# AlerianEmperor/CaitlynRenderer

Measured on AMD Instinct MI355X. Metric: Mray/s (primary+1 bounce) at 1920x1080, higher is better.
Workload: dtype f32

## Files before the change

caitlynrenderer_amd/csrc/crt_device.cpp:

```cpp
#include <hip/hip_runtime.h>
#include <dlfcn.h>

#include <algorithm>
#include <atomic>
#include <chrono>
#include <cmath>
#include <cstdio>
#include <cstdlib>
#include <cstring>
#include <memory>
#include <mutex>
#include <thread>
#include <new>
#include <string>
#include <vector>

#include "../../include/crt.h"
#include "crt_error.hpp"
#include "device_build.hpp"
#include "host/cwbvh.hpp"
#include "host/flatnode_link.hpp"
#include "host/refit_core.hpp"
#include "instances.hpp"
#include "instances_bind.hpp"
// ... 154 lines not shown
    uint32_t* d_counts = nullptr;
    uint32_t bank = 0;
    bool counts_clean = false;
    uint32_t* counts() const { return d_counts + (size_t)bank * kCounters; }
    uint32_t* h_counts = nullptr;
    bool frame_buffers_ready = false;

    crt_camera cam{};
    bool have_camera = false;
    uint32_t jitter = 1;
    bool count_visits = false;
    bool count_batched = false;
    unsigned long long* d_visit_totals = nullptr;
    unsigned long long* h_visit_totals = nullptr;

    float4* d_t_rays = nullptr; float4* d_t_hits = nullptr; uint32_t* d_t_stats = nullptr; size_t t_cap = 0;

    std::vector<EventSpan> spans;
    int n_spans = 0;
    crt_frame_stats stats{};
    bool stats_pending = false;
    bool stats_from_frame = false;
    bool stats_counted = false;
    uint32_t tri_min = 2;
    uint32_t inplace_shadow = 3;
    uint32_t accel = 0;
    uint32_t refill_min = 8;
    uint32_t trace_pool = 64;
    uint32_t trace_occupancy = 8;
    uint32_t oversubscribe = 0;
    bool special_materials = false;
    uint32_t waves_per_workgroup = 1;
    uint32_t lanes_per_ray = 8;
    uint32_t* d_overflow = nullptr;
    float4* d_lfinal = nullptr;
    uint32_t ray_bins = 0;
    bool rows_padded = false;
    bool rays_doubled = false;
    uint32_t* d_bins = nullptr;
    float bounds_lo[3] = {0.f, 0.f, 0.f}, bounds_hi[3] = {1.f, 1.f, 1.f};
    uint32_t* bin_count(uint32_t seg) const { return d_bins + (size_t)seg * CRT_RAY_BINS; }
    uint32_t* bin_cap(uint32_t par, uint32_t seg) const { return d_bins + (size_t)(17 + par * 17 + seg) * CRT_RAY_BINS; }
    uint32_t* bin_off(uint32_t par, uint32_t seg) const { return d_bins + (size_t)(17 * 3 + par * 17 + seg) * CRT_RAY_BINS; }
    uint32_t* bin_start(uint32_t seg) const { return d_bins + (size_t)17 * 5 * CRT_RAY_BINS + (size_t)seg * (CRT_RAY_BINS + 1u); }
    uint32_t* bin_ovf(uint32_t seg) const { return d_bins + (size_t)17 * 5 * CRT_RAY_BINS + (size_t)17 * (CRT_RAY_BINS + 1u) + (size_t)seg * 32u; }
    static size_t bins_words() { return (size_t)17 * 5 * CRT_RAY_BINS + (size_t)17 * (CRT_RAY_BINS + 1u) + 17u * 32u; }
    uint32_t debug_fail_batch_alloc = 0;
    uint32_t batch_cap = 1;
    uint32_t samples_in_stats = 1;
    uint32_t timing = 0;
    bool timing_accumulate = false;

    std::vector<crt_scene*> peers;
    crt_scene* primary = nullptr;
    std::vector<std::pair<size_t, size_t>> scene_bufs;
    uint32_t shard_rank = 0, shard_world = 1;
    uint32_t streams = 1;
    bool shares_scene = false;
    std::vector<float*> d_gather;
    std::vector<uint2*> d_peer_tiles;
    std::vector<hipEvent_t> ev_peer;
    void* rccl_lib = nullptr;
    std::vector<void*> rccl_comms;
    uint32_t gather_transport = 0;
    float last_gather_ms = 0.f;

// ... 876 lines not shown
    else if (!std::strcmp(name, "persistent")) s->persistent = value ? 1u : 0u;
    else if (!std::strcmp(name, "sort_shadow")) s->sort_shadow = value ? 1u : 0u;
#ifdef CRT_EXPERIMENTS
    else if (!std::strcmp(name, "trace_occupancy")) s->trace_occupancy = (uint32_t)std::max(1, value);
    else if (!std::strcmp(name, "oversubscribe")) s->oversubscribe = (uint32_t)std::max(0, value);
    else if (!std::strcmp(name, "waves_per_workgroup")) {
        if (value != 1 && value != 2 && value != 4) return fail(CRT_ERR_INVALID, "crt_set_option: waves_per_workgroup is 1, 2 or 4");
        s->waves_per_workgroup = (uint32_t)value;
    }
#else
    else if (!std::strcmp(name, "trace_occupancy") || !std::strcmp(name, "oversubscribe") || !std::strcmp(name, "waves_per_workgroup")) {
        const bool is_default = !std::strcmp(name, "waves_per_workgroup") ? value == 1 : !std::strcmp(name, "oversubscribe") ? value == 0 : true;
        if (!is_default) return fail(CRT_ERR_INVALID, std::string("crt_set_option: ") + name + " is an experimental variant: this library was built without CRT_EXPERIMENTS");
    }
#endif
    else if (!std::strcmp(name, "streams")) {
        if (value < 0 || value > 4) return fail(CRT_ERR_INVALID, "crt_set_option: streams is 0 (pick for me) or 1..4");
        if (value == 0) value = s->info.n_nodes8 < 64 ? 3 : s->max_depth > 1 ? 2 : 1;
        if (s->primary) return fail(CRT_ERR_INVALID, "crt_set_option: streams is set on the scene, not on a replica");
        if ((uint32_t)value == s->streams) return CRT_OK;
        if (s->streams == 1u && !s->peers.empty())
            return fail(CRT_ERR_INVALID, "crt_set_option: streams is for a scene on one device (crt_set_devices already deals its tiles to several)");
        const std::vector<int32_t> ids((size_t)value, (int32_t)s->device);
        const int rc = set_devices_of_shard(s, ids.data(), (uint32_t)value, s->tile ? s->tile : 16u, s->shard_rank, s->shard_world);
        if (rc) return rc;
        s->streams = (uint32_t)value;
        return CRT_OK;
    }
    else if (!std::strcmp(name, "wave_samples")) s->wave_samples = value < 0 ? 0u : std::min<uint32_t>(3u, (uint32_t)value);
    else if (!std::strcmp(name, "wide_first")) s->wide_first = value < 0 ? 0u : std::min<uint32_t>(2u, (uint32_t)value);
    else if (!std::strcmp(name, "lanes_per_ray")) {
        if (value != 1 && value != 8) return fail(CRT_ERR_INVALID, "crt_set_option: lanes_per_ray is 1 or 8");
        s->lanes_per_ray = (uint32_t)value;
    }
    else if (!std::strcmp(name, "inplace_shadow")) {
        if (value < 0 || value > 3) return fail(CRT_ERR_INVALID, "crt_set_option: inplace_shadow is 1 (in place), 0 (every segment's shadow rays deferred), 2 (bounce segments' deferred) or 3 (pick for me)");
        s->inplace_shadow = (uint32_t)value;
    }
    else if (!std::strcmp(name, "adaptive_tiles")) { s->adaptive_tiles = value ? 1u : 0u; if (value) s->tile_state = crt_scene::TILES_WANT; }
    else if (!std::strcmp(name, "accel")) {
        if (value < 0 || value > 2) return fail(CRT_ERR_INVALID, "crt_set_option: accel is 0 (CWBVH), 1 (BVH2, reference order) or 2 (BVH2, lowest-id ties)");
        if (value != 0 && !s->d_bvh2) return fail(CRT_ERR_INVALID, "crt_set_option: the scene was created without a BVH2 (desc.bvh)");
        if (value != 0 && s->special_materials)
            return fail(CRT_ERR_INVALID, "crt_set_option: the BVH2 frame mode is the shipped shader, which is Lambert only; this scene has Mirror / Disney materials");
        s->accel = (uint32_t)value;
    }
    else if (!std::strcmp(name, "timing")) s->timing = (uint32_t)std::max(0, value);
    else if (!std::strcmp(name, "timing_accumulate")) {
        HIPCHK(hipSetDevice(s->device));
        HIPCHK(hipStreamSynchronize(s->stream));
        s->timing_accumulate = value != 0;
        s->n_spans = 0;
        const size_t want = value > 0 ? (size_t)std::min(value, 1 << 14) : 0;
        try { if (s->spans.size() < want) s->spans.resize(want); } catch (const std::exception&) { return fail(CRT_ERR_NOMEM, "crt_set_option: out of host memory (timing spans)"); }
    }
    else if (!std::strcmp(name, "ray_bins")) s->ray_bins = (uint32_t)std::min(5, std::max(0, value));
    else if (!std::strcmp(name, "debug_fail_batch_alloc")) {
        if (value >= 2 && (size_t)(value - 2) < s->peers.size()) s->peers[(size_t)(value - 2)]->debug_fail_batch_alloc = 1u;
        else s->debug_fail_batch_alloc = value == 1 ? 1u : 0u;
        if (value == 0) for (crt_scene* p : s->peers) p->debug_fail_batch_alloc = 0u;
        return CRT_OK;
    }
    else if (!std::strcmp(name, "tri_min")) s->tri_min = (uint32_t)std::min(64, std::max(0, value));
    else if (!std::strcmp(name, "refill_min")) s->refill_min = (uint32_t)std::min(65, std::max(1, value));
    else if (!std::strcmp(name, "trace_pool")) {
        if (value != 64 && value != 128 && value != 256) return fail(CRT_ERR_INVALID, "crt_set_option: trace_pool is 64, 128 or 256");
// ... 211 lines not shown
            HIPCHK(hipMemcpyAsync(s->d_tile_order, s->h_tile_order, nt * sizeof(uint32_t), hipMemcpyHostToDevice, s->stream));
            HIPCHK(hipEventRecord(s->ev_tile_order, s->stream));
            s->tile_order_uploading = true;
            s->tile_state = crt_scene::TILES_DONE;
        }
        ++s->frames_since_tile_measure;
        if (s->tile_state == crt_scene::TILES_WANT && !s->count_visits && (!s->tiles_measured_once || s->frames_since_tile_measure >= 16u)) {
            s->tiles_measured_once = true;
            s->frames_since_tile_measure = 0;
            HIPCHK(hipMemsetAsync(s->d_tile_cost, 0, s->n_local_tiles * sizeof(uint32_t), s->stream));
            measure_tiles = true;
        }
    }
    s->bank ^= 1u;
    if (s->accel == 0u) { const int prc = ensure_planes(s); if (prc) return prc; }
    if (!s->counts_clean) HIPCHK(hipMemsetAsync(s->d_counts, 0, 2 * kCounters * sizeof(uint32_t), s->stream));
    s->counts_clean = false;
    uint32_t* const cnt = s->counts();

    for (uint32_t b = 0; b < s->max_depth; ++b) {
        crt::SegmentArgs sa{};
        sa.nodes = s->d_nodes; sa.planes = s->d_planes; sa.tris = s->d_tris; sa.triangles = s->d_triangles; sa.normals = s->d_normals;
        sa.materials = s->d_materials; sa.lights = s->d_lights; sa.n_lights = (int32_t)s->n_lights;
        sa.stack_entries = s->stack_entries;
        sa.texcoords = s->d_texcoords; sa.textures = s->d_textures;
        sa.tex_width = s->tex_width; sa.tex_height = s->tex_height; sa.n_textures = s->n_textures;
        sa.f = f;
        sa.sub_capacity = s->sub_capacity;
        const bool bvh2 = s->accel != 0u;
        const bool small_tree = s->info.n_nodes8 < 64;
        const bool inplace = b < first_deferred;
        sa.tri_min = small_tree ? 0u : s->tri_min;
        sa.lanes_log2 = s->lanes_per_ray >= 8u ? 3u : s->lanes_per_ray >= 4u ? 2u : s->lanes_per_ray >= 2u ? 1u : 0u;
        sa.nodes2 = s->d_bvh2; sa.tris2 = s->d_tris2; sa.stack_entries2 = s->bvh2_stack; sa.tie = s->accel == 2u ? 1u : 0u;
        const bool bins = uses_ray_bins(s);
        const uint32_t Qe = 8u * s->sub_capacity;
        if (bins && b + 1 < s->max_depth) {
            crt::RayBins& o = sa.bins_out;
            o.count = s->bin_count(b + 1); o.cap = s->bin_cap(s->bank, b + 1); o.off = s->bin_off(s->bank, b + 1);
            o.ovf_count = s->bin_ovf(b + 1); o.ovf_base = Qe;
            o.per_lane = s->ray_bins == 2u ? 1u : s->ray_bins == 3u ? (b > 0 ? 1u : 0u) : s->ray_bins == 4u ? 2u : s->ray_bins == 5u ? (b > 0 ? 2u : 0u) : 0u;
            for (int k = 0; k < 3; ++k) {
                const float ext = s->bounds_hi[k] - s->bounds_lo[k];
                o.origin[k] = s->bounds_lo[k];
                o.scale[k] = ext > 0.f ? 8.0f / ext : 0.f;
            }
        }
        if (bins && b > 0) { sa.bin_start = s->bin_start(b); sa.bin_off_in = s->bin_off(s->bank, b); sa.ovf_base_in = Qe; }
        sa.rays_in = s->d_rays[b & 1]; sa.count_in = cnt + counter_index(b, 0, 0);
        sa.rays_next = s->d_rays[(b + 1) & 1]; sa.count_next = cnt + counter_index(b + 1, 0, 0);
        sa.count_shadow = cnt + counter_index(b, 1, 0);
        if (!inplace) {
            const uint32_t r = b - first_deferred;
            sa.shadow = s->d_nee + 2 * (size_t)r * 8u * s->sub_capacity;
            sa.contrib = s->d_contrib + (size_t)r * n_paths;
            sa.slot_first = (uint32_t)((size_t)r * n_paths);
            sa.slot_bit = 1u << (8u + b);
        }
        sa.pb = s->pb; sa.sum = s->d_sum;
        sa.last_segment = (b + 1 == s->max_depth) ? 1u : 0u;
        sa.visit_totals = s->d_visit_totals;
        sa.overflow = s->d_overflow;
        if (b == 0) { sa.zero_counts = s->d_counts + (size_t)(s->bank ^ 1u) * kCounters; sa.n_zero = kCounters; }
        sa.l_final = folds ? s->d_lfinal : nullptr;
        sa.tile_cost = (b == 0 && measure_tiles) ? s->d_tile_cost : nullptr;
        sa.n_samples = b == 0 ? n_samples : 1u;
// ... 473 lines not shown

}

void crt_scene::drop_peers() {
    if (!rccl_comms.empty() && g_rccl.destroy)
        for (void* c : rccl_comms) if (c) (void)g_rccl.destroy(c);
    rccl_comms.clear();
    for (crt_scene* p : peers) delete p;
    peers.clear();
    if (!d_gather.empty() || !d_peer_tiles.empty() || !ev_peer.empty()) (void)hipSetDevice(device);
    for (float* b : d_gather) if (b) (void)hipFree(b);
    for (uint2* b : d_peer_tiles) if (b) (void)hipFree(b);
    for (hipEvent_t e : ev_peer) if (e) (void)hipEventDestroy(e);
    d_gather.clear(); d_peer_tiles.clear(); ev_peer.clear();
}

static int replicate_scene(const crt_scene* src, int device, crt_scene** out) {
    *out = nullptr;
    HIPCHK(hipSetDevice(device));
    std::unique_ptr<crt_scene> owner(new (std::nothrow) crt_scene);
    crt_scene* r = owner.get();
    if (!r) return fail(CRT_ERR_NOMEM, "crt_set_devices: out of memory");
    r->device = device;
    hipDeviceProp_t prop;
    if (hipGetDeviceProperties(&prop, device) == hipSuccess) r->n_cu = prop.multiProcessorCount;
    HIPCHK(hipStreamCreateWithFlags(&r->stream, hipStreamNonBlocking));
    r->width = src->width; r->height = src->height; r->max_depth = src->max_depth; r->n_lights = src->n_lights;
    r->tex_width = src->tex_width; r->tex_height = src->tex_height; r->n_textures = src->n_textures;
    r->info = src->info; r->bvh2_stack = src->bvh2_stack; r->stack_entries = src->stack_entries; r->special_materials = src->special_materials;
    r->cam = src->cam; r->have_camera = src->have_camera; r->jitter = src->jitter;
    r->tri_min = src->tri_min; r->inplace_shadow = src->inplace_shadow; r->accel = src->accel; r->refill_min = src->refill_min; r->trace_pool = src->trace_pool; r->count_visits = src->count_visits;
    r->count_batched = src->count_batched;
    r->trace_occupancy = src->trace_occupancy; r->oversubscribe = src->oversubscribe; r->waves_per_workgroup = src->waves_per_workgroup;
    r->lanes_per_ray = src->lanes_per_ray; r->bounce_refill = src->bounce_refill; r->refill_pool = src->refill_pool; r->shadow_pool = src->shadow_pool; r->shadow_refill_min = src->shadow_refill_min; r->shadow_waves = src->shadow_waves; r->persistent = src->persistent; r->sort_shadow = src->sort_shadow;
    r->wave_samples = src->wave_samples; r->wide_first = src->wide_first; r->adaptive_tiles = src->adaptive_tiles; r->timing = src->timing;
    r->ray_bins = src->ray_bins; r->rows_padded = src->rows_padded;
    for (int k = 0; k < 3; ++k) { r->bounds_lo[k] = src->bounds_lo[k]; r->bounds_hi[k] = src->bounds_hi[k]; }
    r->scene_bufs = src->scene_bufs;
    r->shares_scene = device == src->device;
    if (device != src->device) {
        int can = 0;
        if (hipDeviceCanAccessPeer(&can, device, src->device) == hipSuccess && can) (void)hipDeviceEnablePeerAccess(src->device, 0);
        (void)hipGetLastError();
    }
    for (const auto& b : src->scene_bufs) {
        const void* from = *reinterpret_cast<void* const*>(reinterpret_cast<const char*>(src) + b.first);
        void** to = reinterpret_cast<void**>(reinterpret_cast<char*>(r) + b.first);
        if (!from) continue;
        if (device == src->device) { *to = const_cast<void*>(from); continue; }
        hipError_t e = hipMalloc(to, b.second ? b.second : 16);
        if (e != hipSuccess) return fail(CRT_ERR_NOMEM, std::string("crt_set_devices: hipMalloc: ") + hipGetErrorString(e));
        if (b.second) HIPCHK(hipMemcpyPeer(*to, device, from, src->device, b.second));
    }
    int rc = finish_scene_setup(r);
    if (rc) return rc;
    *out = owner.release();
    return CRT_OK;
}

int crt_set_devices(crt_scene* s, const int32_t* devices, uint32_t n_devices, uint32_t tile) {
    if (s && s->inst && n_devices > 1)
        return fail(CRT_ERR_INVALID, "crt_set_devices: an instanced scene renders on the one device its crt_instances handle lives on");
    const int rc = set_devices_of_shard(s, devices, n_devices, tile, 0u, 1u);
    if (rc == CRT_OK) { s->shard_rank = 0u; s->shard_world = 1u; }
    return rc;
}

// ... 508 lines not shown
```

caitlynrenderer_amd/csrc/rt_kernels.hip:

```cpp
#include <hip/hip_runtime.h>
#include <hip/hip_ext.h>
#include <stdint.h>

#include <type_traits>
#include <stdlib.h>

#include <algorithm>

#include "rt_kernels.hpp"
#include "rt_math.hpp"
#include "host/flatnode_link.hpp"
#include "rt_traverse.hpp"

namespace crt {

#define CRT_INF 1e9f
#define CRT_EPS 1e-4f
#define CRT_PI 3.1415926f
#define CRT_PI2 6.2831853f


#ifdef CRT_ISA_MARKS
#define CRT_MARK(name) asm volatile("; CRT_MARK " name)
#else
// ... 698 lines not shown
                const uint32_t hitmask = node8_intersect(n0, n1, n2, n3, n4, o, inv, negx, negy, negz, oct4, tmax);
                cur.x = n1.x;
                tg.x = n1.y;
                cur.y = (hitmask & 0xff000000u) | (n0.w >> 24);
                tg.y = hitmask & 0x00ffffffu;
                }
                CRT_MARK("node_end");
            }
            while (tg.y) {
                CRT_MARK("tri_begin");
                const int b = 31 - __builtin_clz(tg.y);
                tg.y &= ~(1u << b);
                const uint32_t ti = tg.x + (uint32_t)b;
                const float4* tp = tri_rows(tris, ti);
                const float4 ta = tp[0], tb = tp[1], tc = tp[2];
                if (STATS) { ++n_tris; count_wave_step(w_tris); }
                float u, v, t;
                if (mt_test(ta, tb, tc, o, d, u, v, t) && t < tmax) { hit_tri = (int)ti; tg.y = 0u; cur.y = 0u; sp = 0; }
                CRT_MARK("tri_end");
            }
            if (!(cur.y & 0xff000000u) && sp != 0) { --sp; cur = stk[sp * 64]; }
        }
    }
    busy = (cur.y & 0xff000000u) != 0u;
    CRT_MARK("loop_end");
    HitState out;
    out.t = tmax; out.tri = hit_tri;
    if (regroup)
        group_phase<true, STATS, false>(nodes, tris, base, stack_entries, overflow, busy, o, d, tmax, -1, cur, tg, sp, tri_min, out, n_nodes, n_tris, w_nodes, w_tris,
                                        V3(0.f, 0.f, 0.f));
    return out.tri >= 0;
}

__device__ __forceinline__ void flush_visit_totals(unsigned long long* totals, uint32_t nn, uint32_t nt, uint32_t wn = 0u, uint32_t wt = 0u) {
    unsigned long long a = nn, b = nt, c = wn, d = wt;
    for (int off = 32; off > 0; off >>= 1) {
        a += __shfl_down(a, off);
        b += __shfl_down(b, off);
        c += __shfl_down(c, off);
        d += __shfl_down(d, off);
    }
    if ((threadIdx.x & 63u) == 0) {
        if (a) atomicAdd(&totals[0], a);
        if (b) atomicAdd(&totals[1], b);
        if (c) atomicAdd(&totals[4], c);
        if (d) atomicAdd(&totals[5], d);
    }
}

template <bool ANY, bool STATS>
__global__ void __launch_bounds__(CRT_TRACE_BLOCK) k_trace(TraceArgs a) {
    extern __shared__ uint2 s_lds[];
    const WaveId wid = wave_id(false, false, a.pool_split_log2);
    const uint32_t lane = wid.lane, wave = wid.wave;
    uint2* stk = s_lds + (size_t)wid.lds_wave * (a.stack_entries + CRT_HIT_SLOTS) * 64u + lane;
    const uint32_t n = a.count_ptr ? *a.count_ptr : a.n;
    uint32_t nn_total = 0, nt_total = 0;
    CRT_CHUNK_LOOP(it) {
        const uint32_t v = static_pool_chunk<true>(wid, nullptr, n, it);
        if (v == CRT_NO_WORK) break;
        const uint32_t pool = 256u >> a.pool_split_log2;
        const uint32_t first = dense_pool_first(v, wave) + wid.sub * pool;
        if (first >= n) continue;
        const uint32_t last = first + pool < n ? first + pool : n;
        uint32_t nn = 0, nt = 0, wn_unused = 0, wt_unused = 0;
        uint32_t nn0 = 0, nt0 = 0;
// ... 292 lines not shown
    float dy = (2.0f * ty - 1.0f) + jy;
    dx = dx * f.aspect_tan;
    dy = dy * f.tan_fov;
    const vec3 right = V3(f.cam_right[0], f.cam_right[1], f.cam_right[2]);
    const vec3 up = V3(f.cam_up[0], f.cam_up[1], f.cam_up[2]);
    const vec3 fwd = V3(f.cam_forward[0], f.cam_forward[1], f.cam_forward[2]);
    d = normalize((right * dx + up * dy) + fwd);
    o = V3(f.cam_pos[0], f.cam_pos[1], f.cam_pos[2]);
}

typedef const __attribute__((address_space(4))) SegmentArgs* KArgs;
__device__ __forceinline__ RayBins load_bins(KArgs k) {
    RayBins b;
    b.count = k->bins_out.count; b.cap = k->bins_out.cap; b.off = k->bins_out.off; b.ovf_count = k->bins_out.ovf_count;
    b.ovf_base = k->bins_out.ovf_base; b.per_lane = k->bins_out.per_lane;
    for (int i = 0; i < 3; ++i) { b.origin[i] = k->bins_out.origin[i]; b.scale[i] = k->bins_out.scale[i]; }
    return b;
}
__device__ __forceinline__ KArgs kernarg_here() {
    KArgs p = (KArgs)__builtin_amdgcn_kernarg_segment_ptr();
    asm volatile("" : "+s"(p));
    return p;
}

#ifndef CRT_SEG_OCC
#define CRT_SEG_OCC 6
#endif
#ifndef CRT_SEG_OCC_DEFERRED
#define CRT_SEG_OCC_DEFERRED 8
#endif
#ifndef CRT_SEG_OCC_FIRST
#define CRT_SEG_OCC_FIRST 6
#endif
#ifndef CRT_SEG_OCC_BATCH
#define CRT_SEG_OCC_BATCH 5
#endif

template <bool FIRST, bool STATS, bool TEX, bool PRETRACED, bool INPLACE, bool BVH2 = false, bool MAT = false, bool BATCH = false, bool WIDE = false, bool ONE = false,
          bool INST = false>
__global__ void __launch_bounds__(CRT_TRACE_BLOCK, ((WIDE || ONE) ? CRT_SEG_OCC_FIRST : (BATCH || STATS) ? CRT_SEG_OCC_BATCH : (!FIRST && !INPLACE && !PRETRACED) ? CRT_SEG_OCC_DEFERRED : CRT_SEG_OCC)) k_segment(std::conditional_t<INST, InstSegmentArgs, SegmentArgs> a) {
    extern __shared__ uint2 s_lds[];
    constexpr bool UNI_K = FIRST;
    const bool wave_samples = BATCH && !WIDE && !ONE && a.wave_samples == 1u;
    const bool lane_samples = BATCH && (ONE || a.wave_samples == 2u);
    const WaveId wid = wave_id(wave_samples, lane_samples);
    const uint32_t lane = wid.lane, wave = wid.wave;
    const uint32_t wave_stride = (a.stack_entries + CRT_HIT_SLOTS) * 64u;
    uint2* stk = s_lds + (size_t)wid.lds_wave * wave_stride + lane;
    int* stk2 = reinterpret_cast<int*>(s_lds) + (size_t)wid.lds_wave * a.stack_entries2 * 64u + lane;
    const float4* const recs = BVH2 ? a.tris2 : a.tris;
    const FrameArgs& f = a.f;
    uint32_t nn = 0, nt = 0, nn_any = 0, nt_any = 0;
    uint32_t wn = 0, wt = 0, wn_any = 0, wt_any = 0;
    uint32_t n_hits = 0;
    uint32_t nu = 0, nu_any = 0;
    if (FIRST && a.zero_counts && blockIdx.x == 0)
        for (uint32_t i = threadIdx.x; i < a.n_zero; i += blockDim.x) a.zero_counts[i] = 0u;
    CRT_CHUNK_LOOP(it) {
        uint32_t v;
        if (!FIRST && a.bin_start) {
            const uint32_t n_chunks = queue_chunks(a.count_in[0]), per_group = (n_chunks + 7u) >> 3;
            const uint32_t grp = wid.vblock & 7u, c = (wid.vblock >> 3) + it * (wid.vgrid >> 3);
            v = (c < per_group && grp * per_group + c < n_chunks) ? (grp << 28) | (grp * per_group + c) : CRT_NO_WORK;
        } else {
            v = static_chunk<FIRST>(wid, a.count_in, f.n_local_pixels, it);
        }
        if (v == CRT_NO_WORK) break;
        const uint32_t g = v >> 28;
        uint32_t* const count_shadow = a.count_shadow + g * CRT_COUNTER_STRIDE;
        uint32_t* const count_next = a.count_next + g * CRT_COUNTER_STRIDE;
        float4* const shadow_q = a.shadow + 2 * (size_t)g * a.sub_capacity;
        float4* const next_q = a.rays_next + 2 * (size_t)g * a.sub_capacity;
        uint32_t e, n;
// ... 293 lines not shown
                            sdir = (ou * dl.x + ov * dl.y) + n * dl.z;
                            bsdf_pdf = __fdiv_rn(dot(sdir, n) * 1.0f, CRT_PI);
                            T = T * albedo;
                        }
                        if (go_on) {
                            if (INPLACE && pending) pend_pdf = bsdf_pdf;
                            else if (INPLACE || FIRST) ka->pb.L[pix] = make_float4(L.x, L.y, L.z, bsdf_pdf);
                            else reinterpret_cast<float*>(ka->pb.L + pix)[3] = bsdf_pdf;
                            ka->pb.T[pix] = make_float4(T.x, T.y, T.z, __uint_as_float((disney ? 2u : 0u) | slot_mask));
                            ka->pb.seed[pix] = make_float2(sx, sy);
                            emit_next = true;
                            finished = false;
                            nx0 = make_float4(hit_point.x, hit_point.y, hit_point.z, CRT_INF);
                            nx1 = make_float4(sdir.x, sdir.y, sdir.z, __uint_as_float(pix));
                        }
                    }
                }
            }
        }
        if (ka->bins_out.count) {
            const RayBins bins_out = load_bins(ka);
            CRT_MARK("loop_begin bins");
            uint32_t* const tab = wave_stride * 8u >= 3072u ? reinterpret_cast<uint32_t*>(s_lds + (size_t)wid.lds_wave * wave_stride) : nullptr;
            const uint32_t ni = bin_append(bins_out, emit_next, ray_bin_key(bins_out, nx0, nx1), tab);
            if (emit_next) { ka->rays_next[2 * (size_t)ni] = nx0; ka->rays_next[2 * (size_t)ni + 1] = nx1; }
            CRT_MARK("loop_end");
        } else {
            const uint32_t ni = wave_append(emit_next, count_next);
            if (emit_next) { next_q[2 * (size_t)ni] = nx0; next_q[2 * (size_t)ni + 1] = nx1; }
        }
        if (INPLACE) {
            const bool lanes_walks = !BVH2 && (ONE || (a.lanes_log2 != 0u && a.tri_min != 0u));
            if (FIRST && lanes_walks) {
                const bool occluded = traverse_any_then_groups<STATS, UNI_K>(a.nodes, a.tris, stk - lane, (int)a.stack_entries, a.overflow, pending, V3(sh0.x, sh0.y, sh0.z),
                                                                      V3(sh1.x, sh1.y, sh1.z), sh0.w, a.tri_min, a.lanes_log2, nn_any, nt_any, wn_any, wt_any, &nu_any, a.planes);
                if (pending && !occluded) L = L + V3(sh2.x, sh2.y, sh2.z);
            } else if (lanes_walks) {
                HitState shh;
                walk_batch<true, STATS, false, UNI_K>(a.nodes, a.tris, stk - lane, (int)a.stack_entries, a.overflow, pending, V3(sh0.x, sh0.y, sh0.z), V3(sh1.x, sh1.y, sh1.z),
                                               sh0.w, a.tri_min, a.lanes_log2, shh, nn_any, nt_any, wn_any, wt_any, V3(0.f, 0.f, 0.f), &nu_any, a.planes);
                if (pending && shh.tri < 0) L = L + V3(sh2.x, sh2.y, sh2.z);
            } else if (pending) {
                HitState sh;
                const vec3 so = V3(sh0.x, sh0.y, sh0.z), sd = V3(sh1.x, sh1.y, sh1.z);
                const bool occluded = BVH2
                    ? traverse_bvh2<true, STATS>(a.nodes2, a.tris2, so, sd, sh0.w, a.tie, stk2, (int)a.stack_entries2, a.overflow, sh, nn_any, nt_any)
                    : traverse<true, STATS, UNI_K>(a.nodes, a.tris, so, sd, sh0.w, stk, (int)a.stack_entries, a.overflow, sh, nn_any, nt_any, wn_any, wt_any, &nu_any);
                if (!occluded) L = L + V3(sh2.x, sh2.y, sh2.z);
            }
            if (pending && emit_next) a.pb.L[pix] = make_float4(L.x, L.y, L.z, pend_pdf);
            pending = false;
        } else {
            const uint32_t si = wave_append(emit_shadow, count_shadow);
            if (emit_shadow) { shadow_q[2 * (size_t)si] = sh0; shadow_q[2 * (size_t)si + 1] = sh1; }
            if (finished) {
                vec3 Lp = V3(0.f, 0.f, 0.f);
                if (!FIRST) { const float4 l = a.pb.L[pix]; Lp = V3(l.x, l.y, l.z); }
                a.l_final[pix] = make_float4(Lp.x, Lp.y, Lp.z, __uint_as_float(0x80000000u | (slot_mask >> 8)));
            }
            finished = false;
        }
        const KArgs kb = kernarg_here();
        if (finished && !pending) {
            if (kb->l_final) kb->l_final[pix] = make_float4(L.x, L.y, L.z, 0.f);
            else if (!wave_samples && !lane_samples && (L.x != 0.f || L.y != 0.f || L.z != 0.f)) add_to_sum(kb->sum, (FIRST && BATCH) ? e : pix, L);
        }
        if (lane_samples && !kb->l_final) {
            const bool mine = finished && !pending;
// ... 211 lines not shown
}
static inline size_t stack_bytes(uint32_t entries) { return (size_t)(entries + CRT_HIT_SLOTS) * 64 * sizeof(uint2); }
static inline dim3 grid_dim(uint32_t grid, uint32_t waves) { return dim3(grid * (4u / waves)); }
static inline dim3 block_dim(uint32_t waves) { return dim3(waves * 64u); }

void launch_trace(const TraceArgs& a_in, int mode, bool stats, uint32_t grid, uint32_t waves, hipStream_t stream) {
    waves = fit_waves(waves, stack_bytes(a_in.stack_entries));
    TraceArgs a = a_in;
    if (waves != 1u || a.pool_split_log2 > 2u) a.pool_split_log2 = 0u;
    const dim3 g = grid_dim(grid << a.pool_split_log2, waves), b = block_dim(waves);
    const size_t lds = waves * stack_bytes(a.stack_entries);
    if (mode == 1) {
        if (stats) launch(k_trace<true, true>, g, b, lds, stream, a);
        else       launch(k_trace<true, false>, g, b, lds, stream, a);
    } else {
        if (stats) launch(k_trace<false, true>, g, b, lds, stream, a);
        else       launch(k_trace<false, false>, g, b, lds, stream, a);
    }
}
void launch_trace_bvh2(const Bvh2Args& a, int any, bool stats, uint32_t grid, uint32_t waves, hipStream_t stream) {
    const size_t per_wave = (size_t)a.stack_entries * 64 * sizeof(int);
    waves = fit_waves(waves, per_wave);
    const dim3 g = grid_dim(grid, waves), b = block_dim(waves);
    const size_t lds = waves * per_wave;
    if (any) {
        if (stats) launch(k_trace_bvh2<true, true>, g, b, lds, stream, a);
        else       launch(k_trace_bvh2<true, false>, g, b, lds, stream, a);
    } else {
        if (stats) launch(k_trace_bvh2<false, true>, g, b, lds, stream, a);
        else       launch(k_trace_bvh2<false, false>, g, b, lds, stream, a);
    }
}
#define CRT_K(F, S, T, P, Y, B2, M, BA, WI, ON) k_segment<F, S, T, P, Y, B2, M, BA, WI, ON>
int launch_segment(const SegmentArgs& a, bool first, bool pretraced, bool inplace, bool bvh2, bool mat, bool stats, uint32_t grid, uint32_t waves, hipStream_t stream) {
    const bool tex = a.textures != nullptr;
    const size_t per_wave = std::max(stack_bytes(a.stack_entries), bvh2 ? (size_t)a.stack_entries2 * 64 * sizeof(int) : (size_t)0);
    waves = fit_waves(waves, per_wave);
    const dim3 g = grid_dim(grid, waves), b = block_dim(waves);
    const size_t lds = waves * per_wave;
    const int feat = tex ? 2 : mat ? 1 : 0;
    if (first && a.n_samples > 1u) {
        const uint32_t ws_passes = (a.n_samples + 3u) / 4u, ws = (a.n_samples + ws_passes - 1u) / ws_passes;
        const size_t lds4 = ws * per_wave + ws * 64 * sizeof(float4);
        SegmentArgs v = a;
        if (a.wave_samples && lds4 > 64u * 1024u) v.wave_samples = 0u;
        if (v.wave_samples == 2u && ((a.n_samples & 3u) || waves != 1u)) v.wave_samples = 0u;
        const bool side_by_side = v.wave_samples == 1u, in_lanes = v.wave_samples == 2u;
        const dim3 gg = side_by_side ? dim3(grid * 4u) : in_lanes ? dim3(grid * 16u) : g, bb = side_by_side ? dim3(ws * 64u) : in_lanes ? dim3(64u) : b;
        const size_t ll = side_by_side ? lds4 : in_lanes ? per_wave : lds;
        const bool one_pass = in_lanes && a.n_samples == 4u && a.tri_min != 0u && a.lanes_log2 != 0u;
        if (stats && one_pass) { launch(CRT_K(true, true, true, false, true, false, true, true, false, true), gg, bb, ll, stream, v); return 2; }
        if (feat == 2 && one_pass)      { launch(CRT_K(true, false, true, false, true, false, true, true, false, true), gg, bb, ll, stream, v); return 2; }
        else if (feat == 1 && one_pass) { launch(CRT_K(true, false, false, false, true, false, true, true, false, true), gg, bb, ll, stream, v); return 2; }
        else if (feat == 2) launch(CRT_K(true, false, true, false, true, false, true, true, false, false), gg, bb, ll, stream, v);
        else if (feat == 1) launch(CRT_K(true, false, false, false, true, false, true, true, false, false), gg, bb, ll, stream, v);
        else if (v.wide_first && one_pass) { launch(CRT_K(true, false, false, false, true, false, false, true, true, true), gg, bb, ll, stream, v); return 3; }
        else if (v.wide_first && !side_by_side) { launch(CRT_K(true, false, false, false, true, false, false, true, true, false), gg, bb, ll, stream, v); return 1; }
        else                launch(CRT_K(true, false, false, false, true, false, false, true, false, false), gg, bb, ll, stream, v);
        return 0;
    }
    if (bvh2) {
        if (first) { if (stats) launch(CRT_K(true, true, true, false, true, true, false, false, false, false), g, b, lds, stream, a);
                     else       launch(CRT_K(true, false, true, false, true, true, false, false, false, false), g, b, lds, stream, a); }
        else       { if (stats) launch(CRT_K(false, true, true, false, true, true, false, false, false, false), g, b, lds, stream, a);
                     else       launch(CRT_K(false, false, true, false, true, true, false, false, false, false), g, b, lds, stream, a); }
        return 0;
    }
    if (pretraced) {
        if (inplace) { if (stats) launch(CRT_K(false, true, true, true, true, false, true, false, false, false), g, b, lds, stream, a);
                       else       launch(CRT_K(false, false, true, true, true, false, true, false, false, false), g, b, lds, stream, a); }
        else         { if (stats) launch(CRT_K(false, true, true, true, false, false, true, false, false, false), g, b, lds, stream, a);
                       else       launch(CRT_K(false, false, true, true, false, false, true, false, false, false), g, b, lds, stream, a); }
        return 0;
    }
    if (!inplace) {
        if (first) { if (stats) launch(CRT_K(true, true, true, false, false, false, true, false, false, false), g, b, lds, stream, a);
                     else       launch(CRT_K(true, false, true, false, false, false, true, false, false, false), g, b, lds, stream, a); }
        else if (stats) launch(CRT_K(false, true, true, false, false, false, true, false, false, false), g, b, lds, stream, a);
        else if (feat == 2) launch(CRT_K(false, false, true, false, false, false, true, false, false, false), g, b, lds, stream, a);
        else if (feat == 1) launch(CRT_K(false, false, false, false, false, false, true, false, false, false), g, b, lds, stream, a);
        else                launch(CRT_K(false, false, false, false, false, false, false, false, false, false), g, b, lds, stream, a);
        return 0;
    }
    if (stats) {
        if (first) launch(CRT_K(true, true, true, false, true, false, true, false, false, false), g, b, lds, stream, a);
        else       launch(CRT_K(false, true, true, false, true, false, true, false, false, false), g, b, lds, stream, a);
        return 0;
    }
    if (feat == 2)      { if (first) launch(CRT_K(true, false, true, false, true, false, true, false, false, false), g, b, lds, stream, a);
                          else       launch(CRT_K(false, false, true, false, true, false, true, false, false, false), g, b, lds, stream, a); }
    else if (feat == 1) { if (first) launch(CRT_K(true, false, false, false, true, false, true, false, false, false), g, b, lds, stream, a);
                          else       launch(CRT_K(false, false, false, false, true, false, true, false, false, false), g, b, lds, stream, a); }
    else                { if (first) launch(CRT_K(true, false, false, false, true, false, false, false, false, false), g, b, lds, stream, a);
                          else       launch(CRT_K(false, false, false, false, true, false, false, false, false, false), g, b, lds, stream, a); }
    return 0;
}
#undef CRT_K
void launch_raygen(const RaygenArgs& a, hipStream_t stream) {
    hipLaunchKernelGGL(k_raygen, dim3((a.f.n_local_pixels + 255u) / 256u), dim3(256), 0, stream, a);
}
void launch_segment_instanced(const InstSegmentArgs& a, bool stats, uint32_t grid, uint32_t waves, hipStream_t stream) {
    waves = fit_waves(waves, stack_bytes(a.stack_entries));
    const dim3 g = grid_dim(grid, waves), b = block_dim(waves);
    const size_t lds = waves * stack_bytes(a.stack_entries);
    if (stats) launch(k_segment<false, true, true, true, false, false, true, false, false, false, true>, g, b, lds, stream, a);
    else       launch(k_segment<false, false, true, true, false, false, true, false, false, false, true>, g, b, lds, stream, a);
}
void launch_closest_queue(const QueueTraceArgs& a, bool stats, uint32_t grid_waves, hipStream_t stream) {
    const dim3 g(grid_waves), b(64u);
    if (stats) launch(k_closest_queue<true>, g, b, stack_bytes(a.stack_entries), stream, a);
    else       launch(k_closest_queue<false>, g, b, stack_bytes(a.stack_entries), stream, a);
}
void launch_nee_sort(const NeeSortArgs& a, uint32_t blocks, hipStream_t stream) {
    hipLaunchKernelGGL(k_nee_hist, dim3(blocks), dim3(256), 0, stream, a);
    hipLaunchKernelGGL(k_nee_scan, dim3(1), dim3(1024), 0, stream, a);
    hipLaunchKernelGGL(k_nee_scatter, dim3(blocks), dim3(256), 0, stream, a);
}
void launch_shadow_deferred(const ShadowArgs& a, bool stats, uint32_t grid_waves, hipStream_t stream) {
    const dim3 g(grid_waves), b(64u);
    if (stats) launch(k_shadow_deferred<true>, g, b, stack_bytes(a.stack_entries), stream, a);
    else       launch(k_shadow_deferred<false>, g, b, stack_bytes(a.stack_entries), stream, a);
}
void launch_bin_scan(const BinScanArgs& a, hipStream_t stream) {
    hipLaunchKernelGGL(k_bin_scan, dim3(1), dim3(1024), 0, stream, a);
}
void launch_fold_paths(float* sum, const float4* l_final, const float4* contrib, uint32_t n_pixels, uint32_t n_samples, uint32_t first_slot_segment, hipStream_t stream) {
    hipLaunchKernelGGL(k_fold_paths, dim3((n_pixels + 255u) / 256u), dim3(256), 0, stream, sum, l_final, contrib, n_pixels, n_samples, first_slot_segment);
}
void launch_untile(const FrameArgs& f, const float* packed, float* linear, uint32_t grid, hipStream_t stream) {
    hipLaunchKernelGGL(k_untile, dim3(grid), dim3(256), 0, stream, f, packed, linear);
// ... 22 lines not shown
```

caitlynrenderer_amd/csrc/rt_kernels.hpp:

```cpp
#pragma once
#include <hip/hip_runtime.h>
#include <stdint.h>

namespace crt {

#define CRT_STACK_ENTRIES 16
#ifndef CRT_HIT_SLOTS
#define CRT_HIT_SLOTS 2
#endif
#ifndef CRT_NODE_ROWS
#define CRT_NODE_ROWS 5
#endif
#ifndef CRT_TRI_ROWS
#define CRT_TRI_ROWS 3
#endif
#define CRT_TRACE_BLOCK 256

struct TraceArgs {
    const uint4* nodes;
    const float4* tris;
    const float4* rays;
    float4* hits;
    uint32_t* stats;
    const uint32_t* count_ptr;
    uint32_t n;
    uint32_t out_orig_id;
    uint32_t stack_entries;
    uint32_t refill_min;
    uint32_t tri_min;
    uint32_t* overflow;
    uint32_t pool_split_log2;
};

struct Bvh2Args {
// ... 63 lines not shown
    FrameArgs f;
    uint32_t sub_capacity;
    uint32_t tri_min;
    uint32_t lanes_log2;
    const float4* rays_in;
    const uint32_t* count_in;
    const float4* hits_in;
    float4* rays_next;   uint32_t* count_next;
    float4* shadow;      uint32_t* count_shadow;
    float4* contrib;
    uint32_t slot_first;
    uint32_t slot_bit;
    PathBuffers pb;
    float* sum;
    uint32_t last_segment;
    unsigned long long* visit_totals;
    const float4* nodes2;
    const float4* tris2;
    uint32_t stack_entries2;
    uint32_t tie;
    uint32_t* zero_counts;
    uint32_t n_zero;
    uint32_t* overflow;
    float4* l_final;
    uint32_t* tile_cost;
    uint32_t wide_first;
    uint32_t wave_samples;
    uint32_t n_samples;
    float rv_s[8];
    RayBins bins_out;
    const uint32_t* bin_start;
    const uint32_t* bin_off_in;
    uint32_t ovf_base_in;
};
struct InstSegmentArgs : SegmentArgs {
    const int32_t* hit_inst;
    const float* inst_w2o;
    const uint2* inst_mesh;
    const uint4* mesh_base;
};

struct RaygenArgs {
    FrameArgs f;
    float4* rays;
    uint32_t* count;
    uint32_t sub_capacity;
    PathBuffers pb;
    uint32_t* zero_counts;
    uint32_t n_zero;
};

struct QueueTraceArgs {
    const uint4* nodes;
    const float4* tris;
    const float4* rays;
    const uint32_t* count;
    float4* hits;
    uint32_t stack_entries;
    uint32_t sub_capacity;
    uint32_t refill_min;
    uint32_t tri_min;
    uint32_t pool;
    uint32_t lanes_log2;
    uint32_t persistent;
    uint32_t* cursors;
    unsigned long long* visit_totals;
    uint32_t* overflow;
// ... 56 lines not shown
```

Before: 17320.

## Defer shadow-ray leaf triangle tests and run them in wave-voted batches

Adds a new any-hit traversal for first-segment shadow rays in the wide one-pass kernel. Each lane parks the leaf triangle groups it finds on the top of its LDS stack instead of testing them right away. A wave-wide ballot then decides whether to run a triangle step or a node step, so lanes stay coherent on one kind of work. It also raises the launch-bounds occupancy target for this variant and spills the shadow contribution into LDS to save registers. The cost is extra LDS traffic and ballot overhead, and parked triangles may delay an early occlusion exit.

```diff
diff --git a/caitlynrenderer_amd/csrc/crt_device.cpp b/caitlynrenderer_amd/csrc/crt_device.cpp
--- a/caitlynrenderer_amd/csrc/crt_device.cpp
+++ b/caitlynrenderer_amd/csrc/crt_device.cpp
@@ -210,6 +210,8 @@
     bool special_materials = false;
     uint32_t waves_per_workgroup = 1;
     uint32_t lanes_per_ray = 8;
+    uint32_t shadow_tri_defer = 3;
+    uint32_t shadow_tri_vote = 32;
     uint32_t* d_overflow = nullptr;
     float4* d_lfinal = nullptr;
     uint32_t ray_bins = 0;
@@ -1152,6 +1154,14 @@
     else if (!std::strcmp(name, "lanes_per_ray")) {
         if (value != 1 && value != 8) return fail(CRT_ERR_INVALID, "crt_set_option: lanes_per_ray is 1 or 8");
         s->lanes_per_ray = (uint32_t)value;
+    }
+    else if (!std::strcmp(name, "shadow_tri_defer")) {
+        if (value < 0 || value > 255) return fail(CRT_ERR_INVALID, "crt_set_option: shadow_tri_defer is 0 (triangles tested in the order found) or the leaf groups a lane may park, 1 .. 255");
+        s->shadow_tri_defer = (uint32_t)value;
+    }
+    else if (!std::strcmp(name, "shadow_tri_vote")) {
+        if (value < 0 || value > 64) return fail(CRT_ERR_INVALID, "crt_set_option: shadow_tri_vote is the share of a wave's live lanes, in 64ths (0 .. 64), that must hold parked triangles for a triangle step");
+        s->shadow_tri_vote = (uint32_t)value;
     }
     else if (!std::strcmp(name, "inplace_shadow")) {
         if (value < 0 || value > 3) return fail(CRT_ERR_INVALID, "crt_set_option: inplace_shadow is 1 (in place), 0 (every segment's shadow rays deferred), 2 (bounce segments' deferred) or 3 (pick for me)");
@@ -1429,6 +1439,7 @@
         const bool inplace = b < first_deferred;
         sa.tri_min = small_tree ? 0u : s->tri_min;
         sa.lanes_log2 = s->lanes_per_ray >= 8u ? 3u : s->lanes_per_ray >= 4u ? 2u : s->lanes_per_ray >= 2u ? 1u : 0u;
+        sa.shadow_tri_defer = s->shadow_tri_defer | (s->shadow_tri_vote << 8);
         sa.nodes2 = s->d_bvh2; sa.tris2 = s->d_tris2; sa.stack_entries2 = s->bvh2_stack; sa.tie = s->accel == 2u ? 1u : 0u;
         const bool bins = uses_ray_bins(s);
         const uint32_t Qe = 8u * s->sub_capacity;
@@ -1968,7 +1979,7 @@
     r->tri_min = src->tri_min; r->inplace_shadow = src->inplace_shadow; r->accel = src->accel; r->refill_min = src->refill_min; r->trace_pool = src->trace_pool; r->count_visits = src->count_visits;
     r->count_batched = src->count_batched;
     r->trace_occupancy = src->trace_occupancy; r->oversubscribe = src->oversubscribe; r->waves_per_workgroup = src->waves_per_workgroup;
-    r->lanes_per_ray = src->lanes_per_ray; r->bounce_refill = src->bounce_refill; r->refill_pool = src->refill_pool; r->shadow_pool = src->shadow_pool; r->shadow_refill_min = src->shadow_refill_min; r->shadow_waves = src->shadow_waves; r->persistent = src->persistent; r->sort_shadow = src->sort_shadow;
+    r->lanes_per_ray = src->lanes_per_ray; r->shadow_tri_defer = src->shadow_tri_defer; r->shadow_tri_vote = src->shadow_tri_vote; r->bounce_refill = src->bounce_refill; r->refill_pool = src->refill_pool; r->shadow_pool = src->shadow_pool; r->shadow_refill_min = src->shadow_refill_min; r->shadow_waves = src->shadow_waves; r->persistent = src->persistent; r->sort_shadow = src->sort_shadow;
     r->wave_samples = src->wave_samples; r->wide_first = src->wide_first; r->adaptive_tiles = src->adaptive_tiles; r->timing = src->timing;
     r->ray_bins = src->ray_bins; r->rows_padded = src->rows_padded;
     for (int k = 0; k < 3; ++k) { r->bounds_lo[k] = src->bounds_lo[k]; r->bounds_hi[k] = src->bounds_hi[k]; }
diff --git a/caitlynrenderer_amd/csrc/rt_kernels.hip b/caitlynrenderer_amd/csrc/rt_kernels.hip
--- a/caitlynrenderer_amd/csrc/rt_kernels.hip
+++ b/caitlynrenderer_amd/csrc/rt_kernels.hip
@@ -754,6 +754,98 @@
     return out.tri >= 0;
 }
 
+template <bool UNI>
+__device__ __forceinline__ bool traverse_any_deferred_then_groups(const uint4* __restrict__ nodes, const float4* __restrict__ tris, uint2* base, int stack_entries,
+                                                                  uint32_t* overflow, bool has_ray, vec3 o, vec3 d, float tmax, uint32_t tri_min, uint32_t max_kl,
+                                                                  uint32_t cap, uint32_t vote, const float4* planes) {
+    constexpr uint32_t KL = GROUP_KL;
+    const uint32_t lane = threadIdx.x & 63u;
+    uint2* const stk = base + lane;
+    const int rows = stack_entries;
+    bool busy = has_ray && __builtin_isfinite(o.x) && __builtin_isfinite(o.y) && __builtin_isfinite(o.z);
+    const vec3 dc = V3(clamp_dir(d.x), clamp_dir(d.y), clamp_dir(d.z));
+    const bool negx = dc.x < 0.0f, negy = dc.y < 0.0f, negz = dc.z < 0.0f;
+    const uint32_t oct4 = (negx ? 0u : 0x04040404u) | (negy ? 0u : 0x02020202u) | (negz ? 0u : 0x01010101u);
+    const vec3 inv = V3(rcp_ieee(dc.x), rcp_ieee(dc.y), rcp_ieee(dc.z));
+    uint2 cur = busy ? make_uint2(0u, 0x80000000u) : make_uint2(0u, 0u);
+    uint2 tg = make_uint2(0u, 0u);
+    int sp = 0, nl = 0;
+    bool regroup = false;
+    CRT_MARK("loop_begin plain");
+    for (;;) {
+        const bool busy_now = (cur.y & 0xff000000u) != 0u, parked = tg.y != 0u;
+        const unsigned long long m_busy = __ballot(busy_now), m_park = __ballot(parked);
+        const uint32_t n_busy = (uint32_t)__builtin_popcountll(m_busy);
+        const bool few = max_kl != 0u && n_busy <= (64u >> KL);
+        bool tri_phase = false;
+        if (m_park == 0ull) {
+            if (n_busy == 0u) break;
+            if (few) { regroup = true; break; }
+        } else {
+            tri_phase = few || n_busy == 0u || (uint32_t)__builtin_popcountll(m_park) * 64u >= vote * (uint32_t)__builtin_popcountll(m_busy | m_park);
+        }
+        const bool full = parked && (nl + 1 >= (int)cap || sp + nl + 2 > rows);
+        if (tri_phase ? parked : (full && busy_now)) {
+            CRT_MARK("tri_begin");
+            const int b = 31 - __builtin_clz(tg.y);
+            tg.y &= ~(1u << b);
+            const uint32_t ti = tg.x + (uint32_t)b;
+            const float4* tp = tri_rows(tris, ti);
+            const float4 ta = tp[0], tb = tp[1], tc = tp[2];
+            float u, v, t;
+            if (mt_test(ta, tb, tc, o, d, u, v, t) && t < tmax) { tg.y = 0u; nl = 0; cur.y = 0u; sp = -1; }
+            else if (tg.y == 0u && nl != 0) { tg = stk[(rows - nl) * 64]; --nl; }
+            CRT_MARK("tri_end");
+        } else if (!tri_phase && busy_now) {
+            CRT_MARK("node_begin");
+            const uint32_t hits_imask = cur.y;
+            const int off = 31 - __builtin_clz(hits_imask);
+            const uint32_t nbase = cur.x;
+            cur.y &= ~(1u << off);
+            if (cur.y & 0xff000000u) { if (sp < stack_entries) { stk[sp * 64] = cur; ++sp; } else atomicAdd(overflow, 1u); }
+            const uint32_t slot = (uint32_t)(off - 24) ^ (oct4 & 0xffu);
+            const uint32_t rel = __builtin_popcount(hits_imask & ~(0xffffffffu << slot));
+            uint32_t key0 = 0u;
+            uint2 ng;
+            if (UNI && node_step_is_uniform(nbase + rel, oct4, key0)) {
+                CRT_MARK("uninode_begin");
+                uint4 n0, n1;
+                const uint32_t oct0 = key0 & 7u;
+                const uint32_t hitmask = node8_intersect_planes(n0, n1, nodes, planes, key0 >> 3, o, inv, oct0, tmax);
+                cur.x = n1.x;
+                ng.x = n1.y;
+                cur.y = (hitmask & 0xff000000u) | (n0.w >> 24);
+                ng.y = hitmask & 0x00ffffffu;
+                CRT_MARK("uninode_end");
+            } else {
+                const uint4* np = node_rows(nodes, nbase + rel);
+                const uint4 n0 = np[0], n1 = np[1], n2 = np[2], n3 = np[3], n4 = np[4];
+                const uint32_t hitmask = node8_intersect(n0, n1, n2, n3, n4, o, inv, negx, negy, negz, oct4, tmax);
+                cur.x = n1.x;
+                ng.x = n1.y;
+                cur.y = (hitmask & 0xff000000u) | (n0.w >> 24);
+                ng.y = hitmask & 0x00ffffffu;
+            }
+            if (ng.y) {
+                if (tg.y == 0u) tg = ng;
+                else { ++nl; stk[(rows - nl) * 64] = ng; }
+            }
+            if (!(cur.y & 0xff000000u) && sp != 0) { --sp; cur = stk[sp * 64]; }
+            CRT_MARK("node_end");
+        }
+    }
+    busy = (cur.y & 0xff000000u) != 0u;
+    CRT_MARK("loop_end");
+    HitState out;
+    out.t = tmax; out.tri = sp < 0 ? 0 : -1;
+    if (regroup) {
+        uint32_t n0 = 0u, n1 = 0u, n2 = 0u, n3 = 0u;
+        group_phase<true, false, false>(nodes, tris, base, stack_entries, overflow, busy, o, d, tmax, -1, cur, make_uint2(0u, 0u), sp, tri_min, out, n0, n1, n2, n3,
+                                        V3(0.f, 0.f, 0.f));
+    }
+    return out.tri >= 0;
+}
+
 __device__ __forceinline__ void flush_visit_totals(unsigned long long* totals, uint32_t nn, uint32_t nt, uint32_t wn = 0u, uint32_t wt = 0u) {
     unsigned long long a = nn, b = nt, c = wn, d = wt;
     for (int off = 32; off > 0; off >>= 1) {
@@ -1112,13 +1204,16 @@
 #ifndef CRT_SEG_OCC_FIRST
 #define CRT_SEG_OCC_FIRST 6
 #endif
+#ifndef CRT_SEG_OCC_ONE
+#define CRT_SEG_OCC_ONE 7
+#endif
 #ifndef CRT_SEG_OCC_BATCH
 #define CRT_SEG_OCC_BATCH 5
 #endif
 
 template <bool FIRST, bool STATS, bool TEX, bool PRETRACED, bool INPLACE, bool BVH2 = false, bool MAT = false, bool BATCH = false, bool WIDE = false, bool ONE = false,
-          bool INST = false>
-__global__ void __launch_bounds__(CRT_TRACE_BLOCK, ((WIDE || ONE) ? CRT_SEG_OCC_FIRST : (BATCH || STATS) ? CRT_SEG_OCC_BATCH : (!FIRST && !INPLACE && !PRETRACED) ? CRT_SEG_OCC_DEFERRED : CRT_SEG_OCC)) k_segment(std::conditional_t<INST, InstSegmentArgs, SegmentArgs> a) {
+          bool INST = false, bool ORDERED = false>
+__global__ void __launch_bounds__(CRT_TRACE_BLOCK, ((WIDE && ONE && !STATS && !ORDERED) ? CRT_SEG_OCC_ONE : (WIDE || ONE) ? CRT_SEG_OCC_FIRST : (BATCH || STATS) ? CRT_SEG_OCC_BATCH : (!FIRST && !INPLACE && !PRETRACED) ? CRT_SEG_OCC_DEFERRED : CRT_SEG_OCC)) k_segment(std::conditional_t<INST, InstSegmentArgs, SegmentArgs> a) {
     extern __shared__ uint2 s_lds[];
     constexpr bool UNI_K = FIRST;
     const bool wave_samples = BATCH && !WIDE && !ONE && a.wave_samples == 1u;
@@ -1478,8 +1573,20 @@
         if (INPLACE) {
             const bool lanes_walks = !BVH2 && (ONE || (a.lanes_log2 != 0u && a.tri_min != 0u));
             if (FIRST && lanes_walks) {
-                const bool occluded = traverse_any_then_groups<STATS, UNI_K>(a.nodes, a.tris, stk - lane, (int)a.stack_entries, a.overflow, pending, V3(sh0.x, sh0.y, sh0.z),
+                bool occluded;
+                if constexpr (WIDE && ONE && !STATS && !ORDERED) {
+                    const uint32_t defer = kernarg_here()->shadow_tri_defer;
+                    uint2* const rec = stk + a.stack_entries * 64u;
+                    rec[0] = make_uint2(__float_as_uint(sh2.x), __float_as_uint(sh2.y));
+                    rec[64].x = __float_as_uint(sh2.z);
+                    occluded = traverse_any_deferred_then_groups<UNI_K>(a.nodes, a.tris, stk - lane, (int)a.stack_entries, a.overflow, pending, V3(sh0.x, sh0.y, sh0.z),
+                                                                        V3(sh1.x, sh1.y, sh1.z), sh0.w, a.tri_min, a.lanes_log2, defer & 0xffu, defer >> 8, a.planes);
+                    const uint2 c01 = rec[0];
+                    sh2 = make_float4(__uint_as_float(c01.x), __uint_as_float(c01.y), __uint_as_float(rec[64].x), 0.f);
+                } else {
+                    occluded = traverse_any_then_groups<STATS, UNI_K>(a.nodes, a.tris, stk - lane, (int)a.stack_entries, a.overflow, pending, V3(sh0.x, sh0.y, sh0.z),
                                                                       V3(sh1.x, sh1.y, sh1.z), sh0.w, a.tri_min, a.lanes_log2, nn_any, nt_any, wn_any, wt_any, &nu_any, a.planes);
+                }
                 if (pending && !occluded) L = L + V3(sh2.x, sh2.y, sh2.z);
             } else if (lanes_walks) {
                 HitState shh;
@@ -1757,6 +1864,7 @@
     }
 }
 #define CRT_K(F, S, T, P, Y, B2, M, BA, WI, ON) k_segment<F, S, T, P, Y, B2, M, BA, WI, ON>
+#define CRT_KD(F, S, T, P, Y, B2, M, BA, WI, ON) (ordered ? k_segment<F, S, T, P, Y, B2, M, BA, WI, ON, false, true> : k_segment<F, S, T, P, Y, B2, M, BA, WI, ON>)
 int launch_segment(const SegmentArgs& a, bool first, bool pretraced, bool inplace, bool bvh2, bool mat, bool stats, uint32_t grid, uint32_t waves, hipStream_t stream) {
     const bool tex = a.textures != nullptr;
     const size_t per_wave = std::max(stack_bytes(a.stack_entries), bvh2 ? (size_t)a.stack_entries2 * 64 * sizeof(int) : (size_t)0);
@@ -1764,6 +1872,7 @@
     const dim3 g = grid_dim(grid, waves), b = block_dim(waves);
     const size_t lds = waves * per_wave;
     const int feat = tex ? 2 : mat ? 1 : 0;
+    const bool ordered = (a.shadow_tri_defer & 0xffu) == 0u;
     if (first && a.n_samples > 1u) {
         const uint32_t ws_passes = (a.n_samples + 3u) / 4u, ws = (a.n_samples + ws_passes - 1u) / ws_passes;
         const size_t lds4 = ws * per_wave + ws * 64 * sizeof(float4);
@@ -1779,7 +1888,7 @@
         else if (feat == 1 && one_pass) { launch(CRT_K(true, false, false, false, true, false, true, true, false, true), gg, bb, ll, stream, v); return 2; }
         else if (feat == 2) launch(CRT_K(true, false, true, false, true, false, true, true, false, false), gg, bb, ll, stream, v);
         else if (feat == 1) launch(CRT_K(true, false, false, false, true, false, true, true, false, false), gg, bb, ll, stream, v);
-        else if (v.wide_first && one_pass) { launch(CRT_K(true, false, false, false, true, false, false, true, true, true), gg, bb, ll, stream, v); return 3; }
+        else if (v.wide_first && one_pass) { launch(CRT_KD(true, false, false, false, true, false, false, true, true, true), gg, bb, ll, stream, v); return 3; }
         else if (v.wide_first && !side_by_side) { launch(CRT_K(true, false, false, false, true, false, false, true, true, false), gg, bb, ll, stream, v); return 1; }
         else                launch(CRT_K(true, false, false, false, true, false, false, true, false, false), gg, bb, ll, stream, v);
         return 0;
@@ -1821,6 +1930,7 @@
     return 0;
 }
 #undef CRT_K
+#undef CRT_KD
 void launch_raygen(const RaygenArgs& a, hipStream_t stream) {
     hipLaunchKernelGGL(k_raygen, dim3((a.f.n_local_pixels + 255u) / 256u), dim3(256), 0, stream, a);
 }
diff --git a/caitlynrenderer_amd/csrc/rt_kernels.hpp b/caitlynrenderer_amd/csrc/rt_kernels.hpp
--- a/caitlynrenderer_amd/csrc/rt_kernels.hpp
+++ b/caitlynrenderer_amd/csrc/rt_kernels.hpp
@@ -1,5 +1,6 @@
 #pragma once
 #include <hip/hip_runtime.h>
+#include <stddef.h>
 #include <stdint.h>
 
 namespace crt {
@@ -129,7 +130,9 @@
     const uint32_t* bin_start;
     const uint32_t* bin_off_in;
     uint32_t ovf_base_in;
-};
+    uint32_t shadow_tri_defer;
+};
+static_assert(sizeof(SegmentArgs) % 8 == 0 && offsetof(SegmentArgs, shadow_tri_defer) + 4 == sizeof(SegmentArgs), "shadow_tri_defer fills the tail padding of SegmentArgs");
 struct InstSegmentArgs : SegmentArgs {
     const int32_t* hit_inst;
     const float* inst_w2o;
```

Measured after the change: 17520, median of 6. 1.01x the previous value.
